# pasqualedem/LabelAnything

Hardware: AMD Instinct MI355X
Metric: episodes/sec (query+support fwd) ViT-B 1024px 1-shot (higher is better)
Workload: dtype f16; 1 GPU; BASELINE cfg2: SAM ViT-B 1024px encoder + LabelAnything decoder, 1-way 1-shot episodes (2 images each), random-init weights, full-resolution logits; parallelism=episode-sharded x1, no collective, launch=hipGraph replay

## Files before the change

### include/la_hip.h

```cpp
#ifndef LA_HIP_H
#define LA_HIP_H
#ifdef __cplusplus
extern "C" {
#endif

enum { LA_F16 = 0, LA_BF16 = 1, LA_F32 = 2, LA_F16X2 = 3 };
enum { LA_ACT_NONE = 0, LA_ACT_GELU = 1, LA_ACT_RELU = 2, LA_ACT_GELU_BWD = 3  };
enum { LA_MAP_NONE = 0, LA_MAP_GROUP = 1, LA_MAP_WINDOW_MERGE = 2, LA_MAP_CONVT2X2 = 3, LA_MAP_WINDOW_PART = 4, LA_MAP_CONV3X3 = 5  };
enum { LA_ATTN_PLAIN = 0, LA_ATTN_RELPOS = 1, LA_ATTN_RELPOS_WIN16 = 2 };

const char* la_last_error(void);
int la_version(void);

int la_gemm_variant(int v);

typedef struct LaGemmEpilogue {
  const float* bias;
  const float* res;
  int ldr;
  int res_mod;
  float* out32;
  int ld32;
  void* out16;
  int ld16;
// ... 136 lines not shown
int la_bilinear_bwd(const float* dy, int n, int oh, int ow, long dy_plane, int dy_ld, float* dx, int ih, int iw, long dx_plane, int dx_ld,
                    void* stream);

int la_bilinear_bwd_set_ok(int oh, int ow, int ih, int iw);
int la_bilinear_bwd_set(const float* dy, int n, int oh, int ow, long dy_plane, int dy_ld, float* dx, int ih, int iw, long dx_plane, int dx_ld,
                        void* stream);

int la_bilinear_rows(const float* in, int N, int h, int w, int C, float* out, int H, int W, void* stream);
int la_bilinear_rows_bwd_set(const float* dy, int n, int oh, int ow, int C, float* dx, int ih, int iw, void* stream);

int la_region_mean_bwd(const float* dy, int B, int M, int C, int g, int k, int D, float* dx, void* stream);

int la_classify_max_bwd(const float* dseg, const float* feat, const float* protos, const int* win, int B, int Npix, int N, int C, int Cf,
                        float* dfeat, float* dprotos, void* stream);

int la_classify_bwd(const float* dseg, const float* feat, const float* protos, int B, int npix, int C, int cf, float* dfeat, float* dprotos,
                    void* stream);

int la_row_broadcast(const float* src, long groups, int rep, int D, float scale, float* out, void* stream);


int la_twoway_pe_layout(const float* table, int hw, int DI, float* out, void* stream);

int la_twoway_t2i(const float* img, const void* wk_hi, const void* wk_lo, const void* wv_hi, const void* wv_lo, const float* pek,
                  const float* bv, const float* q, int G, int hw, int nt, int D, int heads, float* part, float* out, void* stream);

int la_twoway_i2t(float* img, const void* wq_hi, const void* wq_lo, const float* peq, const float* k, const float* v, const void* wo_hi,
                  const void* wo_lo, const float* bo, const float* gamma, const float* beta, float eps, int G, int hw, int nt, int D,
                  int heads, void* stream);


int la_attn_fwd_lse(const void* qkv, const void* vt, void* out16, float* lse, int B, int heads, int T, int Tpad, int E, float scale,
                    int dt, void* stream);

int la_head_transpose(const void* src, int ld, int col0, int B, int heads, int T, int Tpad, void* dst, int dt, void* stream);

int la_attn_bwd(const void* qkv, const void* out16, const void* dout16, const void* kt, const void* qt, const void* dot, float* lse,
                float* dvec, void* dqkv, int B, int heads, int T, int Tpad, int E, float scale, int dt, void* stream);


int la_attn_fwd_relpos_lse(const void* qkv, const void* vt, void* out16, const float* relh, const float* relw, float* lse, int B, int heads,
                           int T, int Tpad, int G, int E, float scale, int dt, void* stream);

int la_attn_bwd_relpos(const void* qkv, const void* out16, const void* dout16, const void* kt, const void* qt, const void* dot, float* lse,
                       float* dvec, void* dqkv, const float* relh, const float* relw, float* drelh, float* drelw, int B, int heads, int T,
                       int Tpad, int G, int E, float scale, int dt, void* stream);

int la_relpos_bwd(const void* qkv, void* dqkv, const float* drelh, const float* drelw, const float* tabh, const float* tabw, float* dtabh,
                  float* dtabw, int B, int heads, int G, int E, float gscale, int dt, void* stream);

int la_cast(const void* src, int src_dt, void* dst, int dst_dt, long n, float scale, void* stream);

int la_transpose16(const void* src, int src_dt, int ld, int R, int C, void* dst, int dst_dt, int Rp, float* colsum, void* stream);

int la_gemm_tn16(const void* dy, int ldy, const void* x, int ldx, float* dw, int lddw, int R, int N, int K, int gsize, int gstride,
                 float* db, int dt, void* stream);

int la_axpy(const float* x, float* y, long n, float a, void* stream);

int la_gelu_fwd16(const void* pre16, void* post16, long n, int dt, void* stream);

int la_gelu_bwd16(const void* pre16, const float* dh, float* d32, void* d16, long n, int dt, void* stream);

int la_qk_fp8(const void* qkv, long rows, int E, void* qk8, int dt, void* stream);
int la_attn_fwd_fp8(const void* qk8, const void* vt, void* out16, int B, int heads, int T, int Tpad, int E, float scale, int dt,
                    void* stream);


int la_colmean16(const void* src, int ld, int groups, int rows_per_group, int D, float* out, float* scratch, int wpart, int H, int W, int dt,
                 void* stream);

int la_layernorm_g(const float* x, const float* xg, int rows_per_group, int ldx, int rows, int E, const float* gamma, const float* beta,
                   float eps, float* out32, void* out16, int window, int H, int W, float* colsum_part, int dt, void* stream);

int la_attn_fwd_cs(const void* qkv, const void* vt, void* out16, const float* relh, const float* relw, const void* tabh, const void* tabw,
                   int B, int heads, int T, int Tpad, int G, int E, float scale, int mode, float* cspart, int csH, int csW, int dt,
                   void* stream);

int la_attn_fwd_rows(const void* qkv, void* out16, const void* tabh, const void* tabw, int B, int heads, int T, int Tpad, int G, int E,
                     float scale, int mode, float* cspart, int imgH, int imgW, const void* padrow, int dt, void* stream);

int la_colsum_fold(const float* part, int groups, int chunks, int D, float inv, float* out, int ldo, void* stream);

int la_add_rowvec(float* x, const float* v, long rows, int rows_per_group, int D, void* stream);
int la_add_rowvec_split(float* x, const float* v, long rows, int rows_per_group, int D, void* split16, void* stream);

int la_norm_finalize(const float* part, int M, int nslots, int E, float eps, float* mr, const void* x16, int ld16, int rows_per_group,
                     float* cs_part, int dt, void* stream);
int la_norm_stats(const float* x, int ldx, int M, int E, float eps, void* x16, float* mr, int dt, void* stream);

int la_error_count(const float* logits, const long long* gt, int B, int C, int H, int W, int ignore_index, unsigned* counts,
                   long long* preds, void* stream);
int la_error_points(const float* logits, const long long* gt, int B, int C, int H, int W, int ignore_index, const unsigned* counts,
                    int num_points, const int* ranks, const float* u, const long long* dims, long dims_stride, int long_side,
                    int custom_preprocess, float* points, float* labels, void* stream);

int la_rle_scan(const int* runs, const int* meta, int K, int* ends, int* area, void* stream);
int la_rle_decode(const int* ends, const int* meta, const int* sel, int k, int H, int W, unsigned char* out, void* stream);
int la_rle_prompt_masks(const int* ends, const int* meta, const int* first, const int* count, const int* index, const int* img_hw,
                        const int* new_hw, int N, int C, int custom, int S, int Mo, float* out, unsigned char* flags, void* stream);
int la_rle_ground_truth(const int* ends, const int* meta, const int* first, const int* count, const int* index, const int* img_hw, int N,
                        int Hmax, int Wmax, long long* out, void* stream);
int la_rle_points(const int* ends, const int* meta, const int* area, const int* new_hw, const int* draws, int D, float* points,
                  unsigned char* flags, void* stream);

int la_classify_wide(const float* tok, const float* img, int B, int Npix, int C, int D, float* seg, void* stream);
int la_classify_wide_bwd(const float* dseg, const float* tok, const float* img, int B, int Npix, int C, int D, float* dimg, float* dtok,
                         void* stream);

int la_level_reduce(const float* cls0, const float* cls1, const float* w, const float* bias, int B, int C, int gh, int gw, float* seg,
                    void* stream);
int la_level_reduce_bwd(const float* dseg, const float* cls0, const float* cls1, const float* w, int B, int C, int gh, int gw, float* dcls0,
                        float* dcls1, float* dw, float* dbias, void* stream);

int la_proto_kernels(const float* protos, const float* W1, const float* W2, int BC, int cf, float* k1, float* K, void* stream);
int la_proto_kernels_bwd(const float* dK, const float* protos, const float* k1, const float* W1, const float* W2, int BC, int cf, float* dk1,
                         float* dprotos, float* dW1, float* dW2, void* stream);

int la_classify_conv(const float* feat, const float* K, int B, int C, int H, int W, int cf, float* seg, void* stream);
int la_classify_conv_bwd(const float* dseg, const float* feat, const float* K, int B, int C, int H, int W, int cf, float* dfeat, float* dK,
                         void* stream);

int la_extract_pool_plan(int M, int hw, int D, int R, int* split_rows, int* nsplit, long long* scratch_floats_per_pair);
int la_extract_pool(const float* x, const float* qt, int qt_broadcast, int B, int M, int C, int hw, int D, int n, float* scratch, float* out,
                    void* stream);
int la_extract_fold(const float* q, const float* Wk, int BC, int n, int D, float* qt, void* stream);
int la_extract_unfold(const float* pooled, const float* Wv, const float* bv, int BC, int n, int D, float* o, void* stream);

#ifdef __cplusplus
}
#endif
#endif
```

### labelanything_amd/_lib.py

```python
from __future__ import annotations

import ctypes as C
import os
from typing import Optional

import torch

_HERE = os.path.dirname(os.path.abspath(__file__))
LIB_PATH = os.path.join(_HERE, "libla_hip.so")

LA_F16, LA_BF16, LA_F32, LA_F16X2 = 0, 1, 2, 3
ACT_NONE, ACT_GELU, ACT_RELU, ACT_GELU_BWD = 0, 1, 2, 3
MAP_NONE, MAP_GROUP, MAP_WINDOW_MERGE, MAP_CONVT2X2, MAP_WINDOW_PART, MAP_CONV3X3 = 0, 1, 2, 3, 4, 5
ATTN_PLAIN, ATTN_RELPOS, ATTN_RELPOS_WIN16 = 0, 1, 2

_DT = {torch.float16: LA_F16, torch.bfloat16: LA_BF16, torch.float32: LA_F32}


class LaGemmEpilogue(C.Structure):
    _fields_ = [
        ("bias", C.c_void_p), ("res", C.c_void_p), ("ldr", C.c_int), ("res_mod", C.c_int),
        ("out32", C.c_void_p), ("ld32", C.c_int), ("out16", C.c_void_p), ("ld16", C.c_int),
        ("act", C.c_int), ("map", C.c_int),
        ("p0", C.c_int), ("p1", C.c_int), ("p2", C.c_int), ("p3", C.c_int), ("p4", C.c_int),
        ("vt", C.c_void_p), ("vt_col0", C.c_int), ("vt_T", C.c_int), ("vt_Tpad", C.c_int),
        ("vt_hd", C.c_int), ("vt_heads", C.c_int), ("vt_ws", C.c_int), ("amap", C.c_int), ("a_kmod", C.c_int), ("ksplit", C.c_int),
        ("aux16", C.c_void_p), ("ldaux", C.c_int),
        ("nstat_out", C.c_void_p), ("rvec", C.c_void_p), ("rvec_rpg", C.c_int), ("nstat_in", C.c_void_p), ("ncol", C.c_void_p),
    ]


_lib: Optional[C.CDLL] = None


def lib() -> C.CDLL:
    global _lib
    if _lib is None:
        if not os.path.exists(LIB_PATH):
            raise RuntimeError(
                f"labelanything_amd: HIP extension {LIB_PATH} is missing - build it with "
                "`python -c 'import __graft_entry__ as g; g.build()'` (there is no CPU/eager fallback)")
        l = C.CDLL(LIB_PATH)
        l.la_last_error.restype = C.c_char_p
        l.la_version.restype = C.c_int
        for name in EXPORTS:
            getattr(l, name).restype = C.c_int
        _lib = l
    return _lib


EXPORTS = [
    "la_gemm", "la_layernorm", "la_im2col_patch", "la_im2col_3x3", "la_relpos_terms", "la_attn_fwd",
    "la_dense_pe", "la_point_embed", "la_mask_embed", "la_attn_small", "la_colmean", "la_class_mean",
    "la_classify", "la_add_cast", "la_conv3x3_f32", "la_nchw_to_nhwc", "la_nhwc_to_nchw", "la_bilinear", "la_post_final",
    "la_confmat_update", "la_resample_u8", "la_u8_to_chw_norm", "la_prompt_masks", "la_focal_loss", "la_adamw_step",
    "la_gemm_tn", "la_gemm_tn16", "la_gemm_fused_act_ok", "la_gemm_plan", "la_colsum_acc", "la_layernorm_bwd", "la_layernorm_bwd_res", "la_transpose_many", "la_act_fwd", "la_act_bwd", "la_attn_small_lse", "la_attn_small_bwd", "la_bilinear_bwd", "la_bilinear_bwd_set", "la_bilinear_bwd_set_ok", "la_bilinear_rows", "la_bilinear_rows_bwd_set",
    "la_classify_bwd", "la_row_broadcast", "la_twoway_t2i", "la_twoway_i2t", "la_gemm_variant", "la_attn_fwd_lse", "la_head_transpose", "la_attn_bwd", "la_cast", "la_gelu_bwd16", "la_axpy", "la_transpose16", "la_qk_fp8", "la_attn_fwd_fp8", "la_colmean16", "la_layernorm_g", "la_add_rowvec", "la_add_rowvec_split", "la_attn_fwd_cs", "la_attn_fwd_rows", "la_colsum_fold", "la_gelu_fwd16", "la_gemm_tn_db",
    "la_attn_fwd_relpos_lse", "la_attn_bwd_relpos", "la_relpos_bwd", "la_twoway_pe_layout",
    "la_norm_finalize", "la_norm_stats", "la_conv3x3_split", "la_conv3x3_split_ok",
    "la_error_count", "la_error_points",
    "la_logits_objective_workspace_bytes", "la_logits_objective", "la_prompt_contrastive_workspace_bytes", "la_prompt_contrastive",
    "la_rle_scan", "la_rle_decode", "la_rle_prompt_masks", "la_rle_ground_truth", "la_rle_points",
    "la_region_mean", "la_classify_max", "la_region_mean_bwd", "la_classify_max_bwd",
    "la_classify_wide", "la_classify_wide_bwd", "la_level_reduce", "la_level_reduce_bwd",
    "la_proto_kernels", "la_proto_kernels_bwd", "la_classify_conv", "la_classify_conv_bwd",
    "la_extract_pool_plan", "la_extract_pool", "la_extract_fold", "la_extract_unfold",
]


def gemm_variant(v: int = -1) -> int:
    return int(lib().la_gemm_variant(int(v)))


def _check(rc: int, what: str) -> None:
    if rc != 0:
        msg = lib().la_last_error().decode()
        raise RuntimeError(f"{what} failed ({rc}): {msg}")


def _ptr(t: Optional[torch.Tensor]):
    return None if t is None else C.c_void_p(t.data_ptr())


def _stream() -> C.c_void_p:
    return C.c_void_p(torch.cuda.current_stream().cuda_stream)


def dt_of(t: torch.Tensor) -> int:
    return _DT[t.dtype]


def _dev(t: torch.Tensor) -> None:
    if not t.is_cuda:
        raise RuntimeError("labelanything_amd kernels need device tensors (no CPU fallback)")
    if t.device.index != torch.cuda.current_device():
        raise RuntimeError(f"tensor on {t.device} but the current device is cuda:{torch.cuda.current_device()}: "
                           "wrap the call in `with torch.cuda.device(tensor.device)`")


class LaGemmPlan(C.Structure):
    _fields_ = [(f, C.c_int) for f in ("kernel", "epi", "planes", "direct", "ragged", "gm", "ksplit", "kchunk", "grid", "block", "lds_bytes")]


GEMM_KERNELS = ("NT", "DMA128", "DMA256x128", "T256", "T256P", "T256Q", "T256W", "F32_N32", "F32_N128", "F32_SMALL", "SKINNY")


def _addr(x) -> Optional[int]:
    return x.data_ptr() if isinstance(x, torch.Tensor) else x


def _gemm_epilogue(m: int, n: int, *, bias=None, res=None, res_mod=0, out32=None, out16=None, act=ACT_NONE, map=MAP_NONE, p=(0, 0, 0, 0, 0), vt=None,
                   vt_col0=0, vt_T=0, vt_Tpad=0, vt_hd=64, vt_heads=0, vt_ws=0, amap=MAP_NONE, a_kmod=0, ksplit=0, aux16=None, nstat_out=None, rvec=None,
                   rvec_rpg=0, nstat_in=None, ncol=None, ldr=None, ld32=None, ld16=None, ldaux=None) -> LaGemmEpilogue:
    def ld(x, given):
        if x is None:
            return 0
        if given is not None:
            return given
        return n if not isinstance(x, torch.Tensor) else (x.stride(-2) if x.dim() >= 2 else 0)

    e = LaGemmEpilogue()
    e.bias, e.res, e.out32, e.out16, e.vt, e.aux16 = _addr(bias), _addr(res), _addr(out32), _addr(out16), _addr(vt), _addr(aux16)
    e.ldr, e.ld32, e.ld16, e.ldaux = ld(res, ldr), ld(out32, ld32), ld(out16, ld16), ld(aux16, ldaux)
    e.res_mod = res_mod
    e.act, e.map = act, map
    e.p0, e.p1, e.p2, e.p3, e.p4 = p
    e.vt_col0, e.vt_T, e.vt_Tpad, e.vt_hd, e.vt_heads = vt_col0, vt_T, vt_Tpad, vt_hd, vt_heads
    e.vt_ws = vt_ws
    e.amap = amap
    e.a_kmod = a_kmod
    e.ksplit = ksplit
    mpad = -(-m // 256) * 256
    if isinstance(nstat_out, torch.Tensor) and (nstat_out.dtype != torch.float32 or nstat_out.numel() < m * (n // 64) * 2):
        raise RuntimeError(f"gemm: nstat_out must be fp32 with at least M * (N / 64) * 2 = {m * (n // 64) * 2} entries")
    if isinstance(nstat_in, torch.Tensor) and (nstat_in.dtype != torch.float32 or nstat_in.numel() < mpad * 2 or ncol is None
                                               or ncol.dtype != torch.float32 or ncol.numel() < n):
        raise RuntimeError(f"gemm: nstat_in must be fp32 [ceil(M / 256) * 256, 2] (>= {mpad * 2} entries) and needs ncol fp32 [N]")
    if isinstance(rvec, torch.Tensor) and (rvec.dtype != torch.float32 or rvec_rpg <= 0 or rvec.numel() < -(-m // rvec_rpg) * n):
        raise RuntimeError("gemm: rvec must be fp32 [ceil(M / rvec_rpg), N] with rvec_rpg > 0")
    e.nstat_out, e.rvec, e.nstat_in, e.ncol = _addr(nstat_out), _addr(rvec), _addr(nstat_in), _addr(ncol)
    e.rvec_rpg = rvec_rpg
    return e


def gemm(a: torch.Tensor, w: torch.Tensor, *, M=None, lda=None, **epilogue) -> None:
    _dev(a)
    m = a.shape[0] if M is None else M
    k = w.shape[1]
    n = w.shape[0]
# ... 633 lines not shown
    _check(lib().la_qk_fp8(_ptr(qkv), C.c_long(qkv.shape[0]), C.c_int(e), _ptr(qk8), C.c_int(dt_of(qkv)), _stream()), "la_qk_fp8")


def add_rowvec_split(x, v, rows_per_group: int, split16) -> None:
    _f32c(x)
    if v is not None:
        _f32c(v)
    if split16.dtype != torch.float16 or tuple(split16.shape) != (x.shape[0], 2 * x.shape[1]) or not split16.is_contiguous():
        raise ValueError("add_rowvec_split: split16 must be a contiguous fp16 [rows, 2 D] buffer")
    _check(lib().la_add_rowvec_split(_ptr(x), _ptr(v), C.c_long(x.shape[0]), C.c_int(rows_per_group), C.c_int(x.shape[1]), _ptr(split16),
                                     _stream()), "la_add_rowvec_split")


def attn_fwd_fp8(qk8, vt, out16, b: int, heads: int, t: int, tpad: int, e: int, scale: float) -> None:
    _dev(qk8)
    _check(lib().la_attn_fwd_fp8(_ptr(qk8), _ptr(vt), _ptr(out16), C.c_int(b), C.c_int(heads), C.c_int(t), C.c_int(tpad), C.c_int(e),
                                 C.c_float(scale), C.c_int(dt_of(out16)), _stream()), "la_attn_fwd_fp8")


def colmean16(src, groups: int, rows_per_group: int, out, scratch, wpart: int = 0, h: int = 0, w: int = 0) -> None:
    _dev(src)
    need = groups * ((rows_per_group + 127) // 128) * src.shape[1]
    if scratch.numel() < need or scratch.dtype != torch.float32:
        raise ValueError(f"colmean16 scratch needs {need} fp32 elements")
    _check(lib().la_colmean16(_ptr(src), C.c_int(src.stride(0)), C.c_int(groups), C.c_int(rows_per_group), C.c_int(src.shape[1]), _ptr(out),
                              _ptr(scratch), C.c_int(wpart), C.c_int(h), C.c_int(w), C.c_int(dt_of(src)), _stream()), "la_colmean16")


LN_CS_ROWS = 32


def ln_cs_chunks(rows_per_group: int) -> int:
    return (rows_per_group + LN_CS_ROWS - 1) // LN_CS_ROWS


def layernorm_g(x, xg, rows_per_group: int, gamma, beta, eps: float, *, out32=None, out16=None, window=0, H=0, W=0, colsum_part=None,
                dt=LA_F16) -> None:
    _dev(x)
    rows, e = x.shape
    if colsum_part is not None:
        need = rows // rows_per_group * ln_cs_chunks(rows_per_group) * e
        if colsum_part.dtype != torch.float32 or colsum_part.numel() < need:
            raise ValueError(f"layernorm_g colsum_part needs {need} fp32 elements")
    _check(lib().la_layernorm_g(_ptr(x), _ptr(xg), C.c_int(rows_per_group), C.c_int(x.stride(0)), C.c_int(rows), C.c_int(e), _ptr(gamma),
                                _ptr(beta), C.c_float(eps), _ptr(out32), _ptr(out16), C.c_int(window), C.c_int(H), C.c_int(W),
                                _ptr(colsum_part), C.c_int(dt), _stream()), "la_layernorm_g")


def attn_fwd_cs(qkv, vt, out16, relh, relw, b: int, heads: int, t: int, tpad: int, g: int, e: int, scale: float, mode: int, cspart,
                cs_h: int = 0, cs_w: int = 0, tabh=None, tabw=None) -> None:
    need = b * ((t + 127) // 128) * e
    if cspart.dtype != torch.float32 or cspart.numel() < need:
        raise ValueError(f"attn_fwd_cs cspart needs {need} fp32 elements")
    _check(lib().la_attn_fwd_cs(_ptr(qkv), _ptr(vt), _ptr(out16), _ptr(relh), _ptr(relw), _ptr(tabh), _ptr(tabw), C.c_int(b), C.c_int(heads),
                                C.c_int(t), C.c_int(tpad), C.c_int(g), C.c_int(e), C.c_float(scale), C.c_int(mode), _ptr(cspart),
                                C.c_int(cs_h), C.c_int(cs_w), C.c_int(dt_of(qkv)), _stream()), "la_attn_fwd_cs")


def attn_fwd_rows(qkv, out16, b: int, heads: int, t: int, tpad: int, g: int, e: int, scale: float, mode: int, tabh=None, tabw=None,
                  cspart=None, img_hw=None, padrow=None) -> None:
    _dev(qkv)
    if qkv.dtype not in (torch.float16, torch.bfloat16) or out16.dtype != qkv.dtype or not (qkv.is_contiguous() and out16.is_contiguous()):
        raise ValueError("attn_fwd_rows: qkv / out16 must be contiguous 16-bit tensors of one dtype")
    if cspart is not None:
        need = b * ((t + 127) // 128) * e
        if cspart.dtype != torch.float32 or cspart.numel() < need:
            raise ValueError(f"attn_fwd_rows cspart needs {need} fp32 elements")
    ih, iw = (0, 0) if img_hw is None else img_hw
    if padrow is not None and (padrow.dtype != qkv.dtype or padrow.numel() != 3 * e or not padrow.is_contiguous()):
        raise ValueError("attn_fwd_rows: padrow must be a contiguous [3E] row of the qkv dtype")
    _check(lib().la_attn_fwd_rows(_ptr(qkv), _ptr(out16), _ptr(tabh), _ptr(tabw), C.c_int(b), C.c_int(heads), C.c_int(t), C.c_int(tpad),
                                  C.c_int(g), C.c_int(e), C.c_float(scale), C.c_int(mode), _ptr(cspart), C.c_int(ih), C.c_int(iw), _ptr(padrow),
                                  C.c_int(dt_of(qkv)), _stream()), "la_attn_fwd_rows")


def colsum_fold(part, groups: int, chunks: int, d: int, inv: float, out) -> None:
    _dev(part)
    if out.dtype != torch.float32 or out.stride(1) != 1 or out.shape[0] < groups or out.shape[1] < d:
        raise ValueError("colsum_fold: out must be fp32 [groups, >= d] with unit column stride")
    _check(lib().la_colsum_fold(_ptr(part), C.c_int(groups), C.c_int(chunks), C.c_int(d), C.c_float(inv), _ptr(out), C.c_int(out.stride(0)),
                                _stream()), "la_colsum_fold")


def add_rowvec(x, v, rows_per_group: int) -> None:
    _f32c(x, v)
    _check(lib().la_add_rowvec(_ptr(x), _ptr(v), C.c_long(x.shape[0]), C.c_int(rows_per_group), C.c_int(x.shape[1]), _stream()), "la_add_rowvec")


def _numel(what: str, **named) -> None:
    for name, (t, n) in named.items():
        if t.numel() != n:
            raise ValueError(f"{what}: {name} must hold {n} elements (got {t.numel()})")


def classify_wide(tok, img, b: int, npix: int, c: int, d: int, seg) -> None:
    _f32c(tok, img, seg)
    _numel("classify_wide", tok=(tok, b * c * d), img=(img, b * npix * d), seg=(seg, b * c * npix))
    _check(lib().la_classify_wide(_ptr(tok), _ptr(img), C.c_int(b), C.c_int(npix), C.c_int(c), C.c_int(d), _ptr(seg), _stream()),
           "la_classify_wide")


def classify_wide_bwd(dseg, tok, img, b: int, npix: int, c: int, d: int, dimg, dtok) -> None:
    _f32c(dseg, tok, img, dimg, dtok)
    _numel("classify_wide_bwd", dseg=(dseg, b * c * npix), tok=(tok, b * c * d), img=(img, b * npix * d), dimg=(dimg, b * npix * d),
           dtok=(dtok, b * c * d))
    _check(lib().la_classify_wide_bwd(_ptr(dseg), _ptr(tok), _ptr(img), C.c_int(b), C.c_int(npix), C.c_int(c), C.c_int(d), _ptr(dimg),
                                      _ptr(dtok), _stream()), "la_classify_wide_bwd")


def level_reduce(cls0, cls1, w, bias, b: int, c: int, gh: int, gw: int, seg) -> None:
    _f32c(cls0, cls1, w, bias, seg)
    _numel("level_reduce", cls0=(cls0, b * c * 16 * gh * gw), cls1=(cls1, b * c * gh * gw), w=(w, 18), bias=(bias, 1),
           seg=(seg, b * c * 16 * gh * gw))
    _check(lib().la_level_reduce(_ptr(cls0), _ptr(cls1), _ptr(w), _ptr(bias), C.c_int(b), C.c_int(c), C.c_int(gh), C.c_int(gw), _ptr(seg),
                                 _stream()), "la_level_reduce")


def level_reduce_bwd(dseg, cls0, cls1, w, b: int, c: int, gh: int, gw: int, dcls0, dcls1, dw, dbias) -> None:
    _f32c(dseg, cls0, cls1, w, dcls0, dcls1, dw, dbias)
    n0, n1 = b * c * 16 * gh * gw, b * c * gh * gw
    _numel("level_reduce_bwd", dseg=(dseg, n0), cls0=(cls0, n0), cls1=(cls1, n1), w=(w, 18), dcls0=(dcls0, n0), dcls1=(dcls1, n1),
           dw=(dw, 18), dbias=(dbias, 1))
    _check(lib().la_level_reduce_bwd(_ptr(dseg), _ptr(cls0), _ptr(cls1), _ptr(w), C.c_int(b), C.c_int(c), C.c_int(gh), C.c_int(gw),
                                     _ptr(dcls0), _ptr(dcls1), _ptr(dw), _ptr(dbias), _stream()), "la_level_reduce_bwd")


def proto_kernels(protos, w1, w2, bc: int, cf: int, k1, k) -> None:
    _f32c(protos, w1, w2, k1, k)
    _numel("proto_kernels", protos=(protos, bc * cf), w1=(w1, 9 * cf * cf), w2=(w2, 9 * cf * cf), k1=(k1, bc * cf * 9), k=(k, bc * 25 * cf))
    _check(lib().la_proto_kernels(_ptr(protos), _ptr(w1), _ptr(w2), C.c_int(bc), C.c_int(cf), _ptr(k1), _ptr(k), _stream()),
           "la_proto_kernels")


def proto_kernels_bwd(dk, protos, k1, w1, w2, bc: int, cf: int, dk1, dprotos, dw1, dw2) -> None:
    _f32c(dk, protos, k1, w1, w2, dk1, dprotos, dw1, dw2)
    _numel("proto_kernels_bwd", dk=(dk, bc * 25 * cf), protos=(protos, bc * cf), k1=(k1, bc * cf * 9), w1=(w1, 9 * cf * cf),
           w2=(w2, 9 * cf * cf), dk1=(dk1, bc * cf * 9), dprotos=(dprotos, bc * cf), dw1=(dw1, 9 * cf * cf), dw2=(dw2, 9 * cf * cf))
    _check(lib().la_proto_kernels_bwd(_ptr(dk), _ptr(protos), _ptr(k1), _ptr(w1), _ptr(w2), C.c_int(bc), C.c_int(cf), _ptr(dk1),
                                      _ptr(dprotos), _ptr(dw1), _ptr(dw2), _stream()), "la_proto_kernels_bwd")


def classify_conv(feat, k, b: int, c: int, h: int, w: int, cf: int, seg) -> None:
    _f32c(feat, k, seg)
    _numel("classify_conv", feat=(feat, b * h * w * cf), k=(k, b * c * 25 * cf), seg=(seg, b * c * h * w))
    _check(lib().la_classify_conv(_ptr(feat), _ptr(k), C.c_int(b), C.c_int(c), C.c_int(h), C.c_int(w), C.c_int(cf), _ptr(seg), _stream()),
           "la_classify_conv")


def classify_conv_bwd(dseg, feat, k, b: int, c: int, h: int, w: int, cf: int, dfeat, dk) -> None:
    _f32c(dseg, feat, k, dfeat, dk)
    _numel("classify_conv_bwd", dseg=(dseg, b * c * h * w), feat=(feat, b * h * w * cf), k=(k, b * c * 25 * cf),
           dfeat=(dfeat, b * h * w * cf), dk=(dk, b * c * 25 * cf))
    _check(lib().la_classify_conv_bwd(_ptr(dseg), _ptr(feat), _ptr(k), C.c_int(b), C.c_int(c), C.c_int(h), C.c_int(w), C.c_int(cf),
                                      _ptr(dfeat), _ptr(dk), _stream()), "la_classify_conv_bwd")


EXTRACT_HEADS = 8


def extract_pool_plan(m: int, hw: int, d: int, r: int):
    split, ns, per = C.c_int(0), C.c_int(0), C.c_longlong(0)
    _check(lib().la_extract_pool_plan(C.c_int(m), C.c_int(hw), C.c_int(d), C.c_int(r), C.byref(split), C.byref(ns), C.byref(per)),
           "la_extract_pool_plan")
    return split.value, ns.value, per.value


# ... 27 lines not shown
```

### labelanything_amd/engine.py

```python
from __future__ import annotations


import math
from typing import Dict, Optional, Tuple

import torch
import torch.nn.functional as F

from . import _lib as L
from .config import LamConfig, EncoderSpec

Tensor = torch.Tensor


def _ceil(a: int, b: int) -> int:
    return (a + b - 1) // b * b


class Arena:

    def __init__(self, device: torch.device):
        self.device = device
        self.bufs: Dict[tuple, Tensor] = {}

    def get(self, name: str, shape, dtype, zero: bool = False, init=None) -> Tensor:
        key = (name, tuple(shape), dtype)
        t = self.bufs.get(key)
        if t is None:
            try:
                t = (torch.zeros if zero else torch.empty)(tuple(shape), device=self.device, dtype=dtype)
            except RuntimeError as e:
                raise RuntimeError(f"HIP out of memory allocating {name}{tuple(shape)}: {e}") from e
            if init is not None:
                init(t)
            self.bufs[key] = t
        return t

    def nbytes(self) -> int:
        return sum(t.numel() * t.element_size() for t in self.bufs.values())


PRECISE_FULL = ("patch", "qkv", "proj", "lin2", "neck")
PRECISE_WIDE = ("patch", "vmean", "projmean", "neck")
PRECISE_WIDE_PLANES = ("patch", "v", "proj", "neck")
PRECISE_DEFAULT = "auto"
PRECISE_GROUPS = ("patch", "qkv", "v", "proj", "lin1", "lin2", "neck", "vmean", "projmean")


_BICUBIC: Dict[tuple, Tensor] = {}


def bicubic_matrix_t(gin: int, gout: int, device) -> Tensor:
    key = (gin, gout, str(device))
    m = _BICUBIC.get(key)
    if m is None:
        eye = torch.eye(gin * gin).view(gin * gin, 1, gin, gin)
        m = F.interpolate(eye, size=(gout, gout), mode="bicubic", align_corners=False).reshape(gin * gin, gout * gout).contiguous().to(device)
        _BICUBIC[key] = m
    return m


def resolve_precise(cfg: LamConfig, precise, dtype: torch.dtype = torch.float16) -> tuple:
    if isinstance(precise, str):
        if precise != "auto":
            raise ValueError("precise must be 'auto', None or a sequence of group names")
        spec = cfg.encoder_spec
        wide = spec is not None and spec.dim >= 512 and dtype == torch.float16
        return PRECISE_WIDE if wide else PRECISE_FULL
    return tuple(precise or ())


class LamEngine:
    def __init__(self, cfg: LamConfig, weights: Dict[str, Tensor], device: torch.device, dtype: torch.dtype = torch.float16,
                 decoder_dtype: Optional[torch.dtype] = torch.float32, precise=PRECISE_DEFAULT, fuse_twoway: bool = True,
                 window_scatter: bool = True, scope: str = "all"):
        if scope not in ("all", "encoder"):
            raise ValueError("scope must be 'all' or 'encoder'")
        self.scope = scope
        if dtype not in (torch.float16, torch.bfloat16):
            raise ValueError("compute dtype must be torch.float16 or torch.bfloat16")
        self.precise = frozenset(resolve_precise(cfg, precise, dtype))
        self.attn_fp8 = False
        self.patch_split = False
        self.isplit = isinstance(decoder_dtype, str) and decoder_dtype == "f16x2"
        if isinstance(decoder_dtype, str):
            if not self.isplit:
                raise ValueError("decoder_dtype must be a torch dtype, None or 'f16x2'")
            decoder_dtype = torch.float32
            self.isplit = cfg.embed_dim % 128 == 0
        if not self.precise <= set(PRECISE_GROUPS):
            raise ValueError(f"unknown precise groups {sorted(self.precise - set(PRECISE_GROUPS))}; known: {PRECISE_GROUPS}")
        self.kmod: Dict[str, int] = {}
        self.mean_kx: Dict[str, int] = {}
        self.fuse_twoway = bool(fuse_twoway) and cfg.embed_dim in (256, 512) and cfg.dec_heads == 8 and decoder_dtype == torch.float32
        self.window_scatter = bool(window_scatter)
        self.attn_rows = True
        self.win_fused_cs = True
        self.conv_implicit = True
        self.conv_split = True
        spec = cfg.encoder_spec
        self.norm_fold = (scope == "all" and spec is not None and dtype == torch.float16 and spec.dim >= 512 and spec.dim % 256 == 0
                          and spec.mlp % 256 == 0 and (3 * spec.heads * 64 * ((spec.head_dim + 63) // 64)) % 256 == 0
                          and not (self.precise & {"qkv", "v", "lin1"}))
        self.norm_fold_packed = self.norm_fold
        self._last16 = None
        self.ddt = dtype if decoder_dtype is None else decoder_dtype
        self.ddti = L._DT[self.ddt]
        L.lib()
        self.cfg = cfg
        self.dev = device
        self.dt = dtype
        self.dti = L._DT[dtype]
        self.arena = Arena(device)
        self.w32: Dict[str, Tensor] = {k: v.detach().to(device=device, dtype=torch.float32).contiguous() for k, v in weights.items()}
        self.p: Dict[str, Tensor] = {}
        self._pe_cache: Dict[int, Tensor] = {}
        self._pe_tables: Dict[tuple, Tensor] = {}
        self._hfpos_cache: Dict[int, Tensor] = {}
        self._pack()

    def _h(self, t: Tensor) -> Tensor:
        return t.to(self.dt).contiguous()

    def _hd(self, t: Tensor) -> Tensor:
        return t.to(self.ddt).contiguous()

    @staticmethod
    def _split3(t: Tensor) -> Tensor:
        hi = t.to(torch.float16)
        lo = (t - hi.float()).to(torch.float16)
        return torch.cat([hi, hi, lo], dim=1).contiguous()

    def ibuf(self, name: str, rows: int, e: int) -> Tensor:
        if self.isplit:
            return self.arena.get(name, (rows, 2 * e), torch.float16, False)
        return self.dbuf(name, (rows, e))

    @property
    def idti(self) -> int:
        return L.LA_F16X2 if self.isplit else self.ddti

    def igemm(self, a: Tensor, wkey: str, **kw) -> None:
        if self.isplit:
            w = self.p[wkey + "s"]
            L.gemm(a, w, a_kmod=2 * (w.shape[1] // 3), **kw)
        else:
            L.gemm(a, self.p[wkey], **kw)

    def _hw(self, key: str, t: Tensor, group: str) -> None:
        t = t.contiguous()
        if group in self.precise and t.shape[1] % 64 == 0:
            hi = t.to(self.dt)
            lo = (t - hi.float()).to(self.dt)
            self.p[key] = torch.cat([hi, lo], dim=1).contiguous()
            self.kmod[key] = t.shape[1]
        else:
            self.p[key] = t.to(self.dt)
            self.kmod.pop(key, None)

    def _pack_fold(self, key: str, wt: Tensor, bias: Tensor, gamma: Tensor, beta: Tensor) -> None:
        wf = (wt * gamma[None, :]).to(self.dt).contiguous()
        self.p[key + "n"] = wf
        self.p[key[:-2] + ".cn"] = wf.double().sum(1).float().contiguous()
        self.p[key[:-2] + ".bn"] = (bias.double() + wt.double() @ beta.double()).float().contiguous()

    def _pack_mean(self, pre: str, wv: Tensor, wo: Tensor, gamma: Optional[Tensor] = None) -> None:
        if gamma is not None and self.norm_fold and self.mean_planes:
            cols = []
            if "vmean" in self.precise:
                wvg = wv * gamma[None, :]
                cols.append((wo.double() @ (wvg - wvg.to(self.dt).float()).double()).float())
            if "projmean" in self.precise:
                cols.append((wo - wo.to(self.dt).float()).float())
            self.p[pre + ".mean.w32n"] = torch.cat(cols, dim=1).contiguous()
        self._pack_mean_plain(pre, wv, wo)

    def _pack_mean_plain(self, pre: str, wv: Tensor, wo: Tensor) -> None:
        cols = []
        if "vmean" in self.precise:
            v_lo = (wv - wv.to(self.dt).float()).double()
# ... 408 lines not shown
                last16 = self._last16 if self._last16 is not None else last16
                continue
            scatter = win16 and "qkv" not in self.precise and arows > rows and self.window_scatter
            if is_global:
                pass
            elif scatter:
                xin = x16
                self.ln(res, bp + ".norm1", 1e-6, out16=xin, **rkw, **ckw)
            else:
                xin = self.buf("enc.xwin", (arows, e), zero=True)
                self.ln(res, bp + ".norm1", 1e-6, out16=xin, window=ws, H=g, W=g, **rkw, **ckw)
            if scatter:
                qb = p[bp + ".qkv.b"]

                def fill_qk(tq, qb=qb):
                    tq[:, : 2 * ea] = qb[: 2 * ea].to(tq.dtype)

                def fill_v(tv, qb=qb):
                    tv.zero_()
                    tv.view(nb, heads, hdp, tpad)[..., : 16 * gg].view(nb, heads, hdp, gg, 16)[..., :gg] = \
                        qb[2 * ea:].view(1, heads, hdp, 1, 1).to(tv.dtype)

                qkv = self.arena.get(f"enc.qkv.w{i}", (arows, 3 * ea), self.dt, False, fill_qk)
                vt = self.arena.get(f"enc.vt.w{i}", (nb * heads, hdp, tpad), self.dt, False, fill_v)
                self.qkv_gemm(xin, bp + ".qkv.w", qkv, vt, ea, rowmap=(L.MAP_WINDOW_PART, (ws, nwy, nwy, g, g)), vt_T=t, vt_Tpad=tpad,
                              vt_hd=hdp, vt_heads=heads, vt_ws=gg)
            else:
                qkv = self.buf("enc.qkv." + tag, (arows, 3 * ea))
                vt = self.buf("enc.vt." + tag, (nb * heads, hdp, tpad), zero=True)
                self.qkv_gemm(xin, bp + ".qkv.w", qkv, vt, ea, vt_T=t, vt_Tpad=tpad, vt_hd=hdp, vt_heads=heads, vt_ws=gg if win16 else 0)
            ao = self.buf("enc.ao." + tag, (arows, ea))
            fused_o = opart is not None and not win16 and gg > 16
            okw = dict(cspart=opart) if fused_o else None

            def attn(relh, relw, mode, **tk):
                if okw is not None:
                    L.attn_fwd_cs(qkv, vt, ao, relh, relw, nb, heads, t, tpad, gg, ea, scale, mode, **okw, **tk)
                else:
                    L.attn_fwd(qkv, vt, ao, relh, relw, nb, heads, t, tpad, gg, ea, scale, mode, **tk)

            if win16:
                attn(None, None, L.ATTN_RELPOS_WIN16, tabh=p[bp + ".tabh"], tabw=p[bp + ".tabw"])
            elif gg <= 16 or gg == 64:
                attn(None, None, L.ATTN_RELPOS, tabh=p[bp + ".tabh"], tabw=p[bp + ".tabw"])
            else:
                relh = self.f32("enc.relh." + tag, (nb * heads, t, gg))
                relw = self.f32("enc.relw." + tag, (nb * heads, t, gg))
                L.relpos_terms(qkv, nb, heads, gg, ea, p[bp + ".tabh"], p[bp + ".tabw"], relh, relw)
                attn(relh, relw, L.ATTN_RELPOS)
            if rvec is not None:
                self.mean_fix(bp, xpart, opart, rvec, bn, hw, o_chunks if fused_o else 0, e, ea, ao=ao,
                              ao_win=(0, 0) if is_global else (ws, g))
            if is_global:
                self.gemm_w(ao, bp + ".proj.w", bias=w[bp + ".attn.proj.bias"], res=res, out32=res)
            else:
                self.gemm_w(ao, bp + ".proj.w", bias=w[bp + ".attn.proj.bias"], res=res, out32=res, M=rows,
                            amap=L.MAP_WINDOW_PART, p=(ws, nwy, nwy, g, g))
            self._sam_mlp(bp, i, res, x16, rows, spec, w, rvec, rkw)
            last16 = self._last16 if self._last16 is not None else last16
        xs = None
        split_neck = self.cfg.use_vit_sam_neck and (pre + ".neck.0.ws") in p
        if split_neck:
            xs = self.buf("enc.res_split", (rows, 2 * e), torch.float16)
            L.add_rowvec_split(res, rvec, hw, xs)
        elif rvec is not None:
            L.add_rowvec(res, rvec, hw)
        if rvec is not None and not (self.cfg.use_vit_sam_neck and "neck" in self.precise):
            last16 = self.buf("enc.last16", (rows, e))
            L.add_cast(res, out16=last16, dt=self.dti)
        if not self.cfg.use_vit_sam_neck:
            return (res, last16, e) if not want_last_block else ((res, last16, e), res)
        out = self.conv_neck(pre + ".neck", last16, bn, g, "enc.neck", x32=res, xs=xs)
        if want_last_block:
            return (out, None, spec.out_chans), res
        return out, None, spec.out_chans

    def _fold_bufs(self, tag: str, rows: int, e: int):
        return self.f32(tag + ".npart", (rows, e // 64, 2)), self.f32(tag + ".nmr", (_ceil(rows, 256), 2), zero=True)

    def _fold_mean(self, pre: str, xpart, opart, bn: int, rpg: int, o_chunks: int, e: int, ea: int, ao) -> Optional[Tensor]:
        if not self.mean_planes:
            return None
        wm = self.p[pre + ".mean.w32n"]
        bar = self.f32("mean.bar", (bn, wm.shape[1]))
        kx = self.mean_kx[pre]
        if xpart is not None:
            L.colsum_fold(xpart, bn, L.norm_cs_chunks(rpg), e, 1.0 / rpg, bar[:, :kx])
        if opart is not None and o_chunks > 0:
            L.colsum_fold(opart, bn, o_chunks, ea, 1.0 / rpg, bar[:, kx:])
        elif opart is not None:
            obar = self.f32("mean.obar", (bn, ea))
            L.colmean16(ao, bn, rpg, obar, opart, 0, 0, 0)
            bar[:, kx:].copy_(obar)
        dr = self.f32("mean.dr", (bn, e))
        L.gemm(bar, wm, out32=dr)
        return dr

    def _planes_to_f32(self, xs: Tensor, name: str) -> Tensor:
        e = xs.shape[1] // 2
        out = self.f32(name, (xs.shape[0], e))
        out.copy_(xs[:, :e])
        out.add_(xs[:, e:])
        return out

    def _sam_encoder_fold(self, images: Tensor, want_last_block: bool = False):
        spec: EncoderSpec = self.cfg.encoder_spec
        pre = "image_encoder"
        bn, _, s, _ = images.shape
        e, heads, g, ws = spec.dim, spec.heads, s // spec.patch, spec.window
        hw = g * g
        rows = bn * hw
        scale = spec.head_dim ** -0.5
        hdp = self.head_pad
        ea = heads * hdp
        w, p = self.w32, self.p
        a, akw = self.patches("enc.patchA", images, rows, spec.patch)
        xs = self.buf("enc.xs", (rows, 2 * e), torch.float16)
        hi, lo = xs[:, :e], xs[:, e:]
        part, mr = self._fold_bufs("enc", rows, e)
        have_mr = False
        if hw % 256 == 0:
            L.gemm(a, p[pre + ".patch.w"], bias=w[pre + ".patch_embed.proj.bias"], res=p[pre + ".pos"], res_mod=hw, out16=hi, aux16=lo,
                   nstat_out=part, **akw)
        else:
            res32 = self.f32("enc.res", (rows, e))
            L.gemm(a, p[pre + ".patch.w"], bias=w[pre + ".patch_embed.proj.bias"], res=p[pre + ".pos"], res_mod=hw, out32=res32, **akw)
            L.add_rowvec_split(res32, None, hw, xs)
            L.norm_stats(res32, 1e-6, self.buf("enc.x16", (rows, e)), mr)
            have_mr = True
        nwy = (g + ws - 1) // ws
        vm, pm = "vmean" in self.precise, "projmean" in self.precise
        for i in range(spec.depth):
            bp = f"{pre}.blocks.{i}"
            is_global = i in spec.global_idx
            o_chunks = _ceil(hw, 128) // 128 if is_global else nwy * nwy * (_ceil(ws * ws, 128) // 128)
            xpart = self.f32("mean.xpart", (bn * L.ln_cs_chunks(hw) * e,)) if vm else None
            opart = self.f32("mean.opart", (bn * max(o_chunks, _ceil(hw, 128) // 128) * ea,)) if pm else None
            if vm or not have_mr:
                L.norm_finalize(None if have_mr else part, rows, e, 1e-6, mr, x16=hi if vm else None, rpg=hw, cs_part=xpart)
            have_mr = False
            qkv = self.buf("enc.qkv.r", (rows, 3 * ea))
            L.gemm(hi, p[bp + ".qkv.wn"], bias=p[bp + ".qkv.bn"], out16=qkv, nstat_in=mr, ncol=p[bp + ".qkv.cn"])
            ao = self.buf("enc.ao.r", (rows, ea))
            fused_o = opart is not None and (is_global or self.win_fused_cs)
            if is_global:
                L.attn_fwd_rows(qkv, ao, bn, heads, hw, _ceil(hw, 64), g, ea, scale, L.ATTN_RELPOS, tabh=p[bp + ".tabh"], tabw=p[bp + ".tabw"],
                                cspart=opart if fused_o else None)
            else:
                L.attn_fwd_rows(qkv, ao, bn * nwy * nwy, heads, ws * ws, _ceil(16 * ws, 64), ws, ea, scale, L.ATTN_RELPOS_WIN16,
                                tabh=p[bp + ".tabh"], tabw=p[bp + ".tabw"], img_hw=(g, g), padrow=p[bp + ".qkv.pad16"],
                                cspart=opart if fused_o else None)
            dr = self._fold_mean(bp, xpart, opart, bn, hw, o_chunks if fused_o else 0, e, ea, ao)
            L.gemm(ao, p[bp + ".proj.w"], bias=w[bp + ".attn.proj.bias"], out16=hi, aux16=lo, nstat_out=part, rvec=dr,
                   rvec_rpg=hw if dr is not None else 0, a_kmod=self.kmod.get(bp + ".proj.w", 0))
            L.norm_finalize(part, rows, e, 1e-6, mr)
            hbuf = self.buf("enc.mlp", (rows, spec.mlp))
            L.gemm(hi, p[bp + ".lin1.wn"], bias=p[bp + ".lin1.bn"], out16=hbuf, act=L.ACT_GELU, nstat_in=mr, ncol=p[bp + ".lin1.cn"])
            L.gemm(hbuf, p[bp + ".lin2.w"], bias=w[bp + ".mlp.lin2.bias"], out16=hi, aux16=lo, nstat_out=part,
                   a_kmod=self.kmod.get(bp + ".lin2.w", 0))
        split_neck = self.cfg.use_vit_sam_neck and (pre + ".neck.0.ws") in p
        res = None
        if want_last_block or not split_neck:
            res = self._planes_to_f32(xs, "enc.res")
        if not self.cfg.use_vit_sam_neck:
            last16 = self.buf("enc.last16", (rows, e))
            last16.copy_(hi)
            return (res, last16, e) if not want_last_block else ((res, last16, e), res)
        out = self.conv_neck(pre + ".neck", hi, bn, g, "enc.neck", x32=res, xs=xs if split_neck else None)
        if want_last_block:
            return (out, None, spec.out_chans), res
        return out, None, spec.out_chans

    def _sam_mlp(self, bp: str, i: int, res: Tensor, x16: Tensor, rows: int, spec, w, rvec, rkw) -> None:
        e = spec.dim
        self.ln(res, bp + ".norm2", 1e-6, out16=x16, **rkw)
        hbuf = self.buf("enc.mlp", (rows, spec.mlp))
        self.gemm_w(x16, bp + ".lin1.w", bias=w[bp + ".mlp.lin1.bias"], out16=hbuf, act=L.ACT_GELU)
# ... 552 lines not shown
```

Before: 392.1 episodes/s.

## Fuse colsum fold and mean-correction GEMM into one persistent kernel with grid barrier

Replaces the two colsum_fold launches plus a small GEMM for the per-group mean correction with a single kernel. It folds the partial column sums into a global scratch buffer, synchronises all blocks with an atomic grid barrier, then computes the small fp32 GEMV-like product. The goal is to cut several tiny kernel launches per encoder block inside the graph. The cost is a spin-based grid barrier that depends on every block being co-resident, with a NaN fallback on timeout, and fp32 FMA summation that replaces the library GEMM.

```diff
diff --git a/include/la_hip.h b/include/la_hip.h
--- a/include/la_hip.h
+++ b/include/la_hip.h
@@ -242,6 +242,10 @@
 
 int la_colsum_fold(const float* part, int groups, int chunks, int D, float inv, float* out, int ldo, void* stream);
 
+int la_mean_fix(const float* xpart, int x_chunks, int kx, const float* opart, int o_chunks, int ko, int groups, float inv_rows,
+                const float* wm, int ldw, int N, float* out, int ldo, void* stream);
+int la_mean_fix_form(int v);
+
 int la_add_rowvec(float* x, const float* v, long rows, int rows_per_group, int D, void* stream);
 int la_add_rowvec_split(float* x, const float* v, long rows, int rows_per_group, int D, void* split16, void* stream);
 
diff --git a/labelanything_amd/_lib.py b/labelanything_amd/_lib.py
--- a/labelanything_amd/_lib.py
+++ b/labelanything_amd/_lib.py
@@ -65,6 +65,7 @@
     "la_classify_wide", "la_classify_wide_bwd", "la_level_reduce", "la_level_reduce_bwd",
     "la_proto_kernels", "la_proto_kernels_bwd", "la_classify_conv", "la_classify_conv_bwd",
     "la_extract_pool_plan", "la_extract_pool", "la_extract_fold", "la_extract_unfold",
+    "la_mean_fix", "la_mean_fix_form",
 ]
 
 
@@ -864,6 +865,31 @@
                                 _stream()), "la_colsum_fold")
 
 
+MEAN_FIX_MAX_GROUPS, MEAN_FIX_MAX_K, MEAN_FIX_MAX_N = 128, 4096, 8064
+
+
+def mean_fix_ok(groups: int, k: int, n: int) -> bool:
+    return 0 < groups <= MEAN_FIX_MAX_GROUPS and 0 < k <= MEAN_FIX_MAX_K and k % 8 == 0 and 0 < n <= MEAN_FIX_MAX_N
+
+
+def mean_fix(xpart, x_chunks: int, kx: int, opart, o_chunks: int, ko: int, groups: int, inv: float, wm, out) -> None:
+    _dev(wm)
+    for name, part, chunks, d in (("xpart", xpart, x_chunks, kx), ("opart", opart, o_chunks, ko)):
+        if part is not None and (part.dtype != torch.float32 or not part.is_contiguous() or part.numel() < groups * chunks * d):
+            raise ValueError(f"mean_fix: {name} must be contiguous fp32 with at least groups * chunks * width = {groups * chunks * d} elements")
+    if wm.dtype != torch.float32 or wm.dim() != 2 or wm.stride(1) != 1 or wm.shape[1] != kx + ko:
+        raise ValueError("mean_fix: wm must be fp32 [N, kx + ko] with unit column stride")
+    if out.dtype != torch.float32 or out.dim() != 2 or out.stride(1) != 1 or out.shape[0] < groups or out.shape[1] < wm.shape[0]:
+        raise ValueError("mean_fix: out must be fp32 [>= groups, >= N] with unit column stride")
+    _check(lib().la_mean_fix(_ptr(xpart), C.c_int(x_chunks), C.c_int(kx), _ptr(opart), C.c_int(o_chunks), C.c_int(ko), C.c_int(groups),
+                             C.c_float(inv), _ptr(wm), C.c_int(wm.stride(0)), C.c_int(wm.shape[0]), _ptr(out), C.c_int(out.stride(0)), _stream()),
+           "la_mean_fix")
+
+
+def mean_fix_form(v: int = -1) -> int:
+    return int(lib().la_mean_fix_form(int(v)))
+
+
 def add_rowvec(x, v, rows_per_group: int) -> None:
     _f32c(x, v)
     _check(lib().la_add_rowvec(_ptr(x), _ptr(v), C.c_long(x.shape[0]), C.c_int(rows_per_group), C.c_int(x.shape[1]), _stream()), "la_add_rowvec")
diff --git a/labelanything_amd/csrc/meanfix.hip b/labelanything_amd/csrc/meanfix.hip
--- /dev/null
+++ b/labelanything_amd/csrc/meanfix.hip
@@ -0,0 +1,167 @@
+#include "la_common.h"
+
+namespace la {
+constexpr int MF_ROWS = 6, MF_COLS = 12;
+constexpr int MF_WAVES = 12, MF_THREADS = MF_WAVES * 64;
+constexpr int MF_MAX_GROUPS = 128;
+constexpr int MF_MAX_K = 4096;
+constexpr unsigned MF_SPIN_LIMIT = 1u << 21;
+
+__device__ float g_mf_bar[MF_MAX_GROUPS * MF_MAX_K];
+__device__ unsigned g_mf_sync[2];
+
+__device__ __forceinline__ void load8(const float* p, float* o) {
+  const float4 a = *reinterpret_cast<const float4*>(p), b = *reinterpret_cast<const float4*>(p + 4);
+  o[0] = a.x; o[1] = a.y; o[2] = a.z; o[3] = a.w; o[4] = b.x; o[5] = b.y; o[6] = b.z; o[7] = b.w;
+}
+
+__global__ __launch_bounds__(MF_THREADS) void mean_fix_kernel(const float* __restrict__ xpart, int x_chunks, int kx, const float* __restrict__ opart,
+                                                              int o_chunks, int ko, int groups, float inv, const float* __restrict__ wm, int ldw,
+                                                              int N, float* __restrict__ out, int ldo, int phases) {
+  __shared__ float part[MF_WAVES][MF_ROWS * MF_COLS][5];
+  __shared__ int s_ok;
+  const int tid = threadIdx.x, lane = tid & 63, wave = __builtin_amdgcn_readfirstlane(tid >> 6);
+  const int K = kx + ko;
+  float* bar = g_mf_bar;
+  if (tid == 0) s_ok = 1;
+  if (phases & 1) {
+    for (int i = blockIdx.x * MF_THREADS + tid; i < groups * K; i += gridDim.x * MF_THREADS) {
+      const int g = i / K, c = i - g * K;
+      const bool isx = c < kx;
+      const int chunks = isx ? x_chunks : o_chunks, D = isx ? kx : ko;
+      const float* p = (isx ? xpart : opart) + (size_t)g * chunks * D + (isx ? c : c - kx);
+      float s0 = 0.f, s1 = 0.f, s2 = 0.f, s3 = 0.f;
+      int j = 0;
+#pragma unroll 4
+      for (; j + 4 <= chunks; j += 4) {
+        s0 += p[(size_t)j * D];
+        s1 += p[(size_t)(j + 1) * D];
+        s2 += p[(size_t)(j + 2) * D];
+        s3 += p[(size_t)(j + 3) * D];
+      }
+      if (j < chunks) s0 += p[(size_t)j * D];
+      if (j + 1 < chunks) s1 += p[(size_t)(j + 1) * D];
+      if (j + 2 < chunks) s2 += p[(size_t)(j + 2) * D];
+      bar[i] = ((s0 + s1) + (s2 + s3)) * inv;
+    }
+  }
+  if (phases == 3) {
+    asm volatile("s_waitcnt vmcnt(0)" ::: "memory");
+    __syncthreads();
+    if (tid == 0) {
+      __builtin_amdgcn_fence(__ATOMIC_RELEASE, "agent");
+      asm volatile("s_waitcnt vmcnt(0)" ::: "memory");
+      __hip_atomic_fetch_add(&g_mf_sync[0], 1u, __ATOMIC_RELAXED, __HIP_MEMORY_SCOPE_AGENT);
+      unsigned spins = 0;
+      while (__hip_atomic_load(&g_mf_sync[0], __ATOMIC_RELAXED, __HIP_MEMORY_SCOPE_AGENT) < gridDim.x) {
+        __builtin_amdgcn_s_sleep(8);
+        if (++spins > MF_SPIN_LIMIT) {
+          s_ok = 0;
+          break;
+        }
+      }
+      __builtin_amdgcn_fence(__ATOMIC_ACQUIRE, "agent");
+      asm volatile("s_waitcnt vmcnt(0)" ::: "memory");
+      if (__hip_atomic_fetch_add(&g_mf_sync[1], 1u, __ATOMIC_RELAXED, __HIP_MEMORY_SCOPE_AGENT) == gridDim.x - 1) {
+        __hip_atomic_store(&g_mf_sync[0], 0u, __ATOMIC_RELAXED, __HIP_MEMORY_SCOPE_AGENT);
+        __hip_atomic_store(&g_mf_sync[1], 0u, __ATOMIC_RELAXED, __HIP_MEMORY_SCOPE_AGENT);
+      }
+    }
+  }
+  __syncthreads();
+  if (!(phases & 2)) return;
+  const bool ok = s_ok != 0;
+  const int kstride = K >= 1024 ? 4 * 512 : 512;
+  const int kw = K >= 1024 ? min(4, (K + 511) / 512) : 1;
+  const int T = MF_WAVES / kw;
+  const int wv = wave % kw, ti = wave / kw;
+  const int ncb = (N + MF_COLS - 1) / MF_COLS, ncu = (ncb + T - 1) / T, nrb = (groups + MF_ROWS - 1) / MF_ROWS;
+  for (int u = blockIdx.x; u < nrb * ncu; u += gridDim.x) {
+    const int cb = (u % ncu) * T + ti, r0 = (u / ncu) * MF_ROWS, n0 = cb * MF_COLS;
+    if (cb < ncb) {
+      float acc[MF_ROWS][MF_COLS];
+#pragma unroll
+      for (int r = 0; r < MF_ROWS; ++r)
+#pragma unroll
+        for (int c = 0; c < MF_COLS; ++c) acc[r][c] = 0.f;
+      for (int k = wv * 512 + lane * 8; k < K; k += kstride) {
+        float x[MF_ROWS][8];
+#pragma unroll
+        for (int r = 0; r < MF_ROWS; ++r) load8(bar + (size_t)min(r0 + r, groups - 1) * K + k, x[r]);
+#pragma unroll
+        for (int c = 0; c < MF_COLS; ++c) {
+          float w[8];
+          load8(wm + (size_t)min(n0 + c, N - 1) * ldw + k, w);
+#pragma unroll
+          for (int r = 0; r < MF_ROWS; ++r)
+#pragma unroll
+            for (int j = 0; j < 8; ++j) acc[r][c] = fmaf(x[r][j], w[j], acc[r][c]);
+        }
+      }
+#pragma unroll
+      for (int r = 0; r < MF_ROWS; ++r)
+#pragma unroll
+        for (int c = 0; c < MF_COLS; ++c) {
+          const float s = row16_sum(acc[r][c]);
+          if ((lane & 15) == 0) part[wave][r * MF_COLS + c][lane >> 4] = s;
+        }
+    }
+    __syncthreads();
+    for (int o = tid; o < T * MF_ROWS * MF_COLS; o += MF_THREADS) {
+      const int t = o / (MF_ROWS * MF_COLS), idx = o - t * (MF_ROWS * MF_COLS);
+      const int row = r0 + idx / MF_COLS, col = ((u % ncu) * T + t) * MF_COLS + idx % MF_COLS;
+      if (row < groups && col < N) {
+        float v = 0.f;
+        for (int w = 0; w < kw; ++w) {
+          const float* p = part[t * kw + w][idx];
+          v += (p[0] + p[1]) + (p[2] + p[3]);
+        }
+        v += 0.f;
+        out[(size_t)row * ldo + col] = ok ? v : __builtin_nanf("");
+      }
+    }
+    __syncthreads();
+  }
+}
+
+static int g_mf_form = 1;
+}
+
+extern "C" int la_mean_fix_form(int v) {
+  const int prev = la::g_mf_form;
+  if (v == 0 || v == 1) la::g_mf_form = v;
+  return prev;
+}
+
+extern "C" int la_mean_fix(const float* xpart, int x_chunks, int kx, const float* opart, int o_chunks, int ko, int groups, float inv_rows,
+                           const float* wm, int ldw, int N, float* out, int ldo, void* stream) {
+  LA_CHECK_ARG(wm && out && (xpart || opart), "la_mean_fix: null pointer (wm, out and at least one of xpart / opart)");
+  LA_CHECK_ARG((xpart ? kx > 0 && x_chunks > 0 : kx == 0) && (opart ? ko > 0 && o_chunks > 0 : ko == 0),
+               "la_mean_fix: a partial buffer needs chunks > 0 and a width > 0, a null one the width 0 (kx=%d x_chunks=%d ko=%d o_chunks=%d)", kx,
+               x_chunks, ko, o_chunks);
+  const int K = kx + ko;
+  LA_CHECK_ARG((K % 8) == 0 && K <= la::MF_MAX_K, "la_mean_fix: kx + ko = %d must be a multiple of 8, at most %d", K, la::MF_MAX_K);
+  LA_CHECK_ARG(groups > 0 && groups <= la::MF_MAX_GROUPS && N > 0 && N <= 8064,
+               "la_mean_fix: 1 <= groups <= %d and N <= 8064 (the shapes la_gemm sums in this order), got groups=%d N=%d", la::MF_MAX_GROUPS, groups, N);
+  LA_CHECK_ARG(ldw >= K && (ldw % 4) == 0 && (reinterpret_cast<uintptr_t>(wm) & 15) == 0 && ldo >= N,
+               "la_mean_fix: ldw >= kx + ko, ldw %% 4 == 0, wm 16-byte aligned, ldo >= N (ldw=%d K=%d ldo=%d N=%d)", ldw, K, ldo, N);
+  hipStream_t st = reinterpret_cast<hipStream_t>(stream);
+  const int kw = K >= 1024 ? ((K + 511) / 512 < 4 ? (K + 511) / 512 : 4) : 1, T = la::MF_WAVES / kw;
+  const int ncb = (N + la::MF_COLS - 1) / la::MF_COLS;
+  const int units = ((groups + la::MF_ROWS - 1) / la::MF_ROWS) * ((ncb + T - 1) / T);
+  const int fold_blocks = (groups * K + la::MF_THREADS - 1) / la::MF_THREADS;
+  const int ncu = la::cu_count();
+  const dim3 blk(la::MF_THREADS);
+  if (la::g_mf_form == 1) {
+    const int want = units > fold_blocks ? units : fold_blocks;
+    hipLaunchKernelGGL(la::mean_fix_kernel, dim3(want < ncu ? want : ncu), blk, 0, st, xpart, x_chunks, kx, opart, o_chunks, ko, groups, inv_rows, wm, ldw,
+                       N, out, ldo, 3);
+  } else {
+    hipLaunchKernelGGL(la::mean_fix_kernel, dim3(fold_blocks < 2 * ncu ? fold_blocks : 2 * ncu), blk, 0, st, xpart, x_chunks, kx, opart, o_chunks, ko,
+                       groups, inv_rows, wm, ldw, N, out, ldo, 1);
+    hipLaunchKernelGGL(la::mean_fix_kernel, dim3(units < 2 * ncu ? units : 2 * ncu), blk, 0, st, xpart, x_chunks, kx, opart, o_chunks, ko, groups,
+                       inv_rows, wm, ldw, N, out, ldo, 2);
+  }
+  LA_CHECK_LAUNCH("la_mean_fix");
+  return 0;
+}
diff --git a/labelanything_amd/engine.py b/labelanything_amd/engine.py
--- a/labelanything_amd/engine.py
+++ b/labelanything_amd/engine.py
@@ -96,6 +96,7 @@
         self.window_scatter = bool(window_scatter)
         self.attn_rows = True
         self.win_fused_cs = True
+        self.mean_fix_fused = True
         self.conv_implicit = True
         self.conv_split = True
         spec = cfg.encoder_spec
@@ -670,8 +671,13 @@
         if not self.mean_planes:
             return None
         wm = self.p[pre + ".mean.w32n"]
+        kx = self.mean_kx[pre]
+        dr = self.f32("mean.dr", (bn, e))
+        if self.mean_fix_fused and (opart is None or o_chunks > 0) and L.mean_fix_ok(bn, wm.shape[1], e):
+            L.mean_fix(xpart, L.norm_cs_chunks(rpg), kx if xpart is not None else 0, opart, o_chunks, ea if opart is not None else 0, bn,
+                       1.0 / rpg, wm, dr)
+            return dr
         bar = self.f32("mean.bar", (bn, wm.shape[1]))
-        kx = self.mean_kx[pre]
         if xpart is not None:
             L.colsum_fold(xpart, bn, L.norm_cs_chunks(rpg), e, 1.0 / rpg, bar[:, :kx])
         if opart is not None and o_chunks > 0:
@@ -680,7 +686,6 @@
             obar = self.f32("mean.obar", (bn, ea))
             L.colmean16(ao, bn, rpg, obar, opart, 0, 0, 0)
             bar[:, kx:].copy_(obar)
-        dr = self.f32("mean.dr", (bn, e))
         L.gemm(bar, wm, out32=dr)
         return dr
 
```

Result: no change. 392.9 episodes/s (median of 2 runs) (+0.2%).
